# YiZhiXiaoGuLI/xerus

Measured on AMD Instinct MI355X. Metric: GFLOP/s on TT contraction + TT-round sweep time, order-10 rank-256, higher is better.
Workload: dtype f64; 1 GPU; TT order-10 n=20 rank-256: <x,y> + x.round(256) per step; order=10, mode_size=20, rank=256, parallelism=replicas x1

## Files before the change

xerus_amd/csrc/smallla.hip:

```cpp
#include "smallla.hpp"

#include "reduce_dev.hpp"

#include <cstdio>

namespace xrs {

constexpr int NB = 32;
typedef double d4 __attribute__((ext_vector_type(4)));
constexpr int PMAX = 512;
constexpr int POT_THREADS = 512;

__device__ __forceinline__ double readlane_d(double v, int l) {
    union { double d; int i[2]; } u;
    u.d = v;
    u.i[0] = __builtin_amdgcn_readlane(u.i[0], l);
    u.i[1] = __builtin_amdgcn_readlane(u.i[1], l);
    return u.d;
}

__device__ __forceinline__ void potrf32_body(double* __restrict__ G, int n, double shift_rel, double* __restrict__ Dinv,
                                             int* __restrict__ status, double* __restrict__ info,
                                             const double* src = nullptr) {
    __shared__ double P[PMAX * (NB + 1)];
    __shared__ double Ds[NB][NB + 1];
    __shared__ double red[16];
    __shared__ int fail;
    const int tid = threadIdx.x, lane = tid & 63, wave = tid >> 6;
    if (src != nullptr && src != G) {
        for (int e = tid; e < n * n; e += POT_THREADS) G[e] = src[e];
        __syncthreads();
    }
    double* dummy = Dinv + size_t(n + 31) * NB + (tid & 31);
    if (tid == 0) fail = 0;
    block_trace<POT_THREADS>(G, n, red);
    const double tr = sum_from_zero<POT_THREADS / 64>(red);
    if (tid == 0 && info) info[0] = tr;
    const double shift = shift_rel * tr;
    if (shift != 0.0)
        for (int i = tid; i < n; i += POT_THREADS) G[size_t(i) * n + i] += shift;
    __syncthreads();
    for (int j0 = 0; j0 < n; j0 += NB) {
        const int jb = min(NB, n - j0);
        for (int e = tid; e < NB * NB; e += POT_THREADS) {
            const int r = e / NB, c = e % NB;
            double v = (r == c) ? 1.0 : 0.0;
            if (r < jb && c < jb && c <= r) v = G[size_t(j0 + r) * n + j0 + c];
            Ds[r][c] = v;
        }
        __syncthreads();
        if (wave == 0) {
            const int r = lane & 31;
            double row[NB];
#pragma unroll
            for (int c = 0; c < NB; ++c) row[c] = Ds[r][c];
            int bad = 0;
#pragma unroll
            for (int k = 0; k < NB; ++k) {
                double dkk = readlane_d(row[k], k);
                const bool okp = (dkk > 0.0) && (dkk < 1.0e300);
                if (!okp && bad == 0 && k < jb) bad = k + 1;
                if (!okp) dkk = 1.0;
                const double d = sqrt(dkk);
                const double inv = 1.0 / d;
                row[k] = (r == k) ? d : ((r > k) ? row[k] * inv : row[k]);
#pragma unroll
                for (int l = k + 1; l < NB; ++l) {
                    const double v = readlane_d(row[k], l);
                    if (r >= l) row[l] -= row[k] * v;
                }
            }
            if (lane < 32) {
#pragma unroll
                for (int c = 0; c < NB; ++c) Ds[r][c] = (c <= r) ? row[c] : 0.0;
            }
            if (lane == 0 && bad && fail == 0) fail = j0 + bad;
        }
        __syncthreads();
        const int t = n - j0 - jb;
        if (wave == 1) {
            const int c = lane & 31;
            double x[NB];
#pragma unroll
            for (int i = 0; i < NB; ++i) x[i] = (i == c) ? 1.0 : 0.0;
#pragma unroll
            for (int k = 0; k < NB; ++k) {
                x[k] = x[k] / Ds[k][k];
// ... 272 lines not shown
        for (int q = 0; q < 4; ++q) {
            const int er = min(max(16 * i + lg + 4 * q, 0), n - 1), ec = min(max(16 * k + lr, 0), n - 1);
            const int row = max(er, ec), col = min(er, ec);
            acc[s][q] = S[size_t(row) * n + col];
        }
    }
#pragma unroll
    for (int s = 0; s < PR_SLOTS; ++s)
#pragma unroll
        for (int q = 0; q < 4; ++q) {
            const int row = 16 * ti[s] + lg + 4 * q, col = 16 * tk[s] + lr;
            const bool inside = ti[s] >= 0 && row < n && col < n;
            const double pad = (row == col) ? 1.0 : 0.0;
            acc[s][q] = inside ? acc[s][q] + ((row == col) ? shift : 0.0) : pad;
        }

    for (int j = 0; j < T; ++j) {
        int oc = (lg * PT + lr) * 8, oa = (lr * PT + lg) * 8;
        asm volatile("" : "+v"(oc), "+v"(oa));
        auto cpos = [&](double* base, int q) -> double* {
            return reinterpret_cast<double*>(reinterpret_cast<char*>(base) + oc) + 4 * q * PT;
        };
        auto apos = [&](const double* base, int c) -> const double* {
            return reinterpret_cast<const double*>(reinterpret_cast<const char*>(base) + oa) + 4 * c;
        };
#pragma unroll
        for (int s = 0; s < PR_SLOTS; ++s)
            if (ti[s] == j && tk[s] == j) {
#pragma unroll
                for (int q = 0; q < 4; ++q) *cpos(Dt, q) = acc[s][q];
            }
        __syncthreads();
        PSTAMP(2 + 4 * j);
        if (wave == 0) {
            const int bad = diag_factor16(Dt, Di, ivs, Dinv + size_t(j) * 256, lane, n - 16 * j);
            if (lane == 0 && bad && fail == 0) fail = 16 * j + bad;
        }
        __syncthreads();
        PSTAMP(3 + 4 * j);
#pragma unroll
        for (int s = 0; s < PR_SLOTS; ++s) {
            if (tk[s] != j) continue;
            if (ti[s] == j) {
#pragma unroll
                for (int q = 0; q < 4; ++q) acc[s][q] = *cpos(Dt, q);
                continue;
            }
            double* Pi = P + ti[s] * PTILE;
#pragma unroll
            for (int q = 0; q < 4; ++q) *cpos(Pi, q) = acc[s][q];
            wave_lds_sync();
            d4 rr = {0.0, 0.0, 0.0, 0.0};
#pragma unroll
            for (int c = 0; c < 4; ++c) rr = __builtin_amdgcn_mfma_f64_16x16x4f64(*apos(Pi, c), *apos(Di, c), rr, 0, 0, 0);
            wave_lds_sync();
#pragma unroll
            for (int q = 0; q < 4; ++q) *cpos(Pi, q) = rr[q];
            acc[s] = rr;
        }
        __syncthreads();
        PSTAMP(4 + 4 * j);
        trail_all<PR_SLOTS - 1>(acc, ti, tk, j, P, oa);
    }
    __syncthreads();
    PSTAMP(1);
    int sg = lg, sr = lr;
    asm volatile("" : "+v"(sg), "+v"(sr));
#pragma unroll
    for (int s = 0; s < PR_SLOTS; ++s) {
        if (ti[s] < 0 || G == nullptr) continue;
#pragma unroll
        for (int q = 0; q < 4; ++q) {
            const int row = 16 * ti[s] + sg + 4 * q, col = 16 * tk[s] + sr;
            if (row < n && col < n) {
                G[size_t(row) * n + col] = (col <= row) ? acc[s][q] : 0.0;
                if (ti[s] != tk[s]) G[size_t(col) * n + row] = 0.0;
            }
        }
    }
    __syncthreads();
    if (tid == 0) status[0] = fail;
}

constexpr int LA_THREADS = PR_THREADS;
constexpr int LA_WAVES = LA_THREADS / 64;
constexpr int LA_SLOTS = PR_SLOTS;

template <int P>
__device__ __forceinline__ void la_trail_pair(d4 (&acc)[LA_SLOTS], const int (&ti)[LA_SLOTS], const int (&tk)[LA_SLOTS],
                                              int kmin, int kmax, const double* Pbuf, int oa) {
    const bool hi = tk[P] >= kmin && tk[P] <= kmax;
    bool lo = false;
    if constexpr (P > 0) lo = tk[P - 1] >= kmin && tk[P - 1] <= kmax;
    if (!hi && !lo) return;
    auto op = [&](int tile, int c) -> double {
        return *reinterpret_cast<const double*>(reinterpret_cast<const char*>(Pbuf + max(tile, 0) * PTILE) + oa + 32 * c);
    };
    double a1[4], b1[4];
#pragma unroll
    for (int c = 0; c < 4; ++c) {
        a1[c] = hi ? -op(ti[P], c) : 0.0;
        b1[c] = hi ? op(tk[P], c) : 0.0;
    }
    if constexpr (P > 0) {
        double a0[4], b0[4];
#pragma unroll
        for (int c = 0; c < 4; ++c) {
            a0[c] = lo ? -op(ti[P - 1], c) : 0.0;
            b0[c] = lo ? op(tk[P - 1], c) : 0.0;
        }
#pragma unroll
        for (int c = 0; c < 4; ++c) {
            acc[P] = __builtin_amdgcn_mfma_f64_16x16x4f64(a1[c], b1[c], acc[P], 0, 0, 0);
            acc[P - 1] = __builtin_amdgcn_mfma_f64_16x16x4f64(a0[c], b0[c], acc[P - 1], 0, 0, 0);
        }
    } else {
#pragma unroll
        for (int c = 0; c < 4; ++c) acc[P] = __builtin_amdgcn_mfma_f64_16x16x4f64(a1[c], b1[c], acc[P], 0, 0, 0);
    }
}

template <int P>
__device__ __forceinline__ void la_trail_all(d4 (&acc)[LA_SLOTS], const int (&ti)[LA_SLOTS], const int (&tk)[LA_SLOTS],
                                             int kmin, int kmax, const double* Pbuf, int oa) {
    if constexpr (P >= 0) {
        la_trail_pair<P>(acc, ti, tk, kmin, kmax, Pbuf, oa);
        la_trail_all<P - 2>(acc, ti, tk, kmin, kmax, Pbuf, oa);
    }
}

__device__ __forceinline__ void potrf_la_body(double* __restrict__ G, int n, double shift_rel, double* __restrict__ Dinv,
                                              int* __restrict__ status, double* __restrict__ info,
                                              const double* __restrict__ src = nullptr) {
    const double* __restrict__ S = src != nullptr ? src : G;
    __shared__ double Dt[PTILE];
    __shared__ double Di[PTILE];
    __shared__ double P[PR_TMAX * PTILE];
    __shared__ double ivs[16];
    __shared__ double red[LA_WAVES];
    __shared__ int fail;
    const int tid = threadIdx.x, lane = tid & 63;
    const int wave = __builtin_amdgcn_readfirstlane(tid >> 6);
    const int lr = lane & 15, lg = lane >> 4;
    const int T = (n + 15) >> 4;
    const int ntiles = T * (T + 1) / 2;
    if (tid == 0) fail = 0;
    PSTAMP(0);
    block_trace<LA_THREADS>(S, n, red);
    const double tr = sum_from_zero<LA_WAVES>(red);
    if (tid == 0 && info) info[0] = tr;
    const double shift = shift_rel * tr;

    int ti[LA_SLOTS], tk[LA_SLOTS];
    d4 acc[LA_SLOTS];
#pragma unroll
    for (int s = 0; s < LA_SLOTS; ++s) {
        const int t = wave == 0 ? s : LA_SLOTS + s * (LA_WAVES - 1) + (wave - 1);
        int i = -1, k = -1;
        if (t < ntiles) {
            int start = 0;
            k = 0;
            while (t >= start + (T - k)) { start += T - k; ++k; }
            i = k + (t - start);
        }
        ti[s] = i;
        tk[s] = k;
#pragma unroll
        for (int q = 0; q < 4; ++q) {
            const int er = min(max(16 * i + lg + 4 * q, 0), n - 1), ec = min(max(16 * k + lr, 0), n - 1);
            const int row = max(er, ec), col = min(er, ec);
            acc[s][q] = S[size_t(row) * n + col];
        }
    }
#pragma unroll
    for (int s = 0; s < LA_SLOTS; ++s)
#pragma unroll
        for (int q = 0; q < 4; ++q) {
            const int row = 16 * ti[s] + lg + 4 * q, col = 16 * tk[s] + lr;
            const bool inside = ti[s] >= 0 && row < n && col < n;
            const double pad = (row == col) ? 1.0 : 0.0;
            acc[s][q] = inside ? acc[s][q] + ((row == col) ? shift : 0.0) : pad;
        }

    int oc = (lg * PT + lr) * 8, oa = (lr * PT + lg) * 8;
    auto cpos = [&](double* base, int q) -> double* {
        return reinterpret_cast<double*>(reinterpret_cast<char*>(base) + oc) + 4 * q * PT;
    };
    auto apos = [&](const double* base, int c) -> const double* {
        return reinterpret_cast<const double*>(reinterpret_cast<const char*>(base) + oa) + 4 * c;
    };
    auto publish_diag = [&](int j) {
#pragma unroll
        for (int s = 0; s < LA_SLOTS; ++s)
            if (ti[s] == j && tk[s] == j) {
#pragma unroll
                for (int q = 0; q < 4; ++q) *cpos(Dt, q) = acc[s][q];
            }
    };
    auto factor_diag = [&](int j) {
        if (wave == 0) {
            const int bad = diag_factor16(Dt, Di, ivs, Dinv + size_t(j) * 256, lane, n - 16 * j);
            if (lane == 0 && bad && fail == 0) fail = 16 * j + bad;
        }
    };
    publish_diag(0);
    __syncthreads();
    factor_diag(0);
    __syncthreads();
    for (int j = 0; j < T; ++j) {
        asm volatile("" : "+v"(oc), "+v"(oa));
        PSTAMP(2 + 4 * j);
#pragma unroll
        for (int s = 0; s < LA_SLOTS; ++s) {
            if (tk[s] != j) continue;
            if (ti[s] == j) {
#pragma unroll
                for (int q = 0; q < 4; ++q) acc[s][q] = *cpos(Dt, q);
                continue;
            }
            double* Pi = P + ti[s] * PTILE;
#pragma unroll
            for (int q = 0; q < 4; ++q) *cpos(Pi, q) = acc[s][q];
            wave_lds_sync();
            d4 rr = {0.0, 0.0, 0.0, 0.0};
#pragma unroll
            for (int c = 0; c < 4; ++c) rr = __builtin_amdgcn_mfma_f64_16x16x4f64(*apos(Pi, c), *apos(Di, c), rr, 0, 0, 0);
            wave_lds_sync();
#pragma unroll
            for (int q = 0; q < 4; ++q) *cpos(Pi, q) = rr[q];
            acc[s] = rr;
        }
        __syncthreads();
        if (j + 1 >= T) break;
        PSTAMP(3 + 4 * j);
        la_trail_all<LA_SLOTS - 1>(acc, ti, tk, j + 1, j + 1, P, oa);
        publish_diag(j + 1);
        __syncthreads();
        PSTAMP(4 + 4 * j);
        if (wave == 0) factor_diag(j + 1);
        la_trail_all<LA_SLOTS - 1>(acc, ti, tk, j + 2, T - 1, P, oa);
        __syncthreads();
    }
    PSTAMP(1);
    int sg = lg, sr = lr;
    asm volatile("" : "+v"(sg), "+v"(sr));
#pragma unroll
    for (int s = 0; s < LA_SLOTS; ++s) {
        if (ti[s] < 0 || G == nullptr) continue;
#pragma unroll
        for (int q = 0; q < 4; ++q) {
            const int row = 16 * ti[s] + sg + 4 * q, col = 16 * tk[s] + sr;
            if (row < n && col < n) {
                G[size_t(row) * n + col] = (col <= row) ? acc[s][q] : 0.0;
                if (ti[s] != tk[s]) G[size_t(col) * n + row] = 0.0;
            }
        }
    }
    __syncthreads();
    if (tid == 0) status[0] = fail;
}

#ifdef XRS_POTRF_NO_LOOKAHEAD
#define XRS_POTRF_RR_BODY potrf_rr_body
#else
#define XRS_POTRF_RR_BODY potrf_la_body
#endif
#define XRS_POTRF_RR_THREADS PR_THREADS
__global__ void __launch_bounds__(XRS_POTRF_RR_THREADS) k_potrf_rr(double* __restrict__ G, int n, double shift_rel,
                                                         double* __restrict__ Dinv, int* __restrict__ status,
                                                         double* __restrict__ info) {
    XRS_POTRF_RR_BODY(G, n, shift_rel, Dinv, status, info);
}

__global__ void __launch_bounds__(POT_THREADS) k_potrf32_batched(PotrfBatch b) {
    const int i = blockIdx.x;
    potrf32_body(b.G[i], b.n[i], b.shift[i], b.Dinv[i], b.status + b.slot[i], nullptr, b.src[i]);
}

__global__ void __launch_bounds__(XRS_POTRF_RR_THREADS) k_potrf_rr_batched(PotrfBatch b) {
    const int i = blockIdx.x;
    XRS_POTRF_RR_BODY(b.G[i], b.n[i], b.shift[i], b.Dinv[i], b.status + b.slot[i], nullptr, b.src[i]);
}

template <bool COLS, int TMAX>
__device__ __forceinline__ void trsm16_body(const double* __restrict__ L, const double* __restrict__ Dinv, int dld,
                                            int n, const double* __restrict__ Y, size_t ldy, double* __restrict__ X,
                                            size_t ldx, int nvec, int v0, bool ident) {
    constexpr int JS = TMAX / 4;
    __shared__ double Xs[TMAX * 16 * PT];
    __shared__ double red[2][4][256];
    const int tid = threadIdx.x, lane = tid & 63;
    const int wave = __builtin_amdgcn_readfirstlane(tid >> 6);
    const int lr = lane & 15, lg = lane >> 4;
    const int T = (n + 15) >> 4;
    const int np = T * 16;
    for (int e = tid; e < np * 16; e += 256) {
        int i, v;
        if (COLS) { i = e >> 4; v = e & 15; } else { v = e / np; i = e - v * np; }
        double y = 0.0;
        if (i < n && v0 + v < nvec) {
            if (ident) y = (i == v0 + v) ? 1.0 : 0.0;
            else y = COLS ? Y[size_t(i) * ldy + v0 + v] : Y[size_t(v0 + v) * ldy + i];
        }
        Xs[i * PT + v] = y;
    }
    auto dinv_at = [&](int I, int c) -> double {
        const int off = (dld == 32) ? 16 * (I & 1) : 0;
        return Dinv[size_t(16 * I + lr) * dld + off + 4 * c + lg];
    };
    d4 xr[JS];
    double la[JS][4], lb[JS][4], da[4], db[4];
#pragma unroll
    for (int js = 0; js < JS; ++js) {
        xr[js] = d4{0.0, 0.0, 0.0, 0.0};
#pragma unroll
        for (int c = 0; c < 4; ++c) la[js][c] = 0.0;
    }
#pragma unroll
    for (int c = 0; c < 4; ++c) da[c] = dinv_at(0, c);
    __syncthreads();
    for (int I = 0; I < T; ++I) {
        if (I + 1 < T) {
            const int row = 16 * (I + 1) + lr;
#pragma unroll
            for (int js = 0; js < JS; ++js) {
                const int J = wave + 4 * js;
#pragma unroll
                for (int c = 0; c < 4; ++c)
                    lb[js][c] = (J <= I && row < n) ? L[size_t(row) * n + 16 * J + 4 * c + lg] : 0.0;
            }
#pragma unroll
            for (int c = 0; c < 4; ++c) db[c] = dinv_at(I + 1, c);
        }
        d4 y;
#pragma unroll
        for (int q = 0; q < 4; ++q) y[q] = Xs[(16 * I + lg + 4 * q) * PT + lr];
        d4 accj[JS];
#pragma unroll
        for (int js = 0; js < JS; ++js) {
            accj[js] = d4{0.0, 0.0, 0.0, 0.0};
            if (wave + 4 * js >= I) continue;
#pragma unroll
            for (int c = 0; c < 4; ++c) accj[js] = __builtin_amdgcn_mfma_f64_16x16x4f64(la[js][c], xr[js][c], accj[js], 0, 0, 0);
        }
        d4 acc = accj[0];
#pragma unroll
        for (int js = 1; js < JS; ++js) acc += accj[js];
        double* rb = red[I & 1][0];
#pragma unroll
        for (int q = 0; q < 4; ++q) rb[wave * 256 + q * 64 + lane] = acc[q];
        __syncthreads();
        d4 t;
#pragma unroll
        for (int q = 0; q < 4; ++q)
            t[q] = y[q] - ((rb[q * 64 + lane] + rb[256 + q * 64 + lane]) + (rb[512 + q * 64 + lane] + rb[768 + q * 64 + lane]));
        d4 x0 = {0.0, 0.0, 0.0, 0.0}, x1 = {0.0, 0.0, 0.0, 0.0};
        x0 = __builtin_amdgcn_mfma_f64_16x16x4f64(da[0], t[0], x0, 0, 0, 0);
        x1 = __builtin_amdgcn_mfma_f64_16x16x4f64(da[1], t[1], x1, 0, 0, 0);
        x0 = __builtin_amdgcn_mfma_f64_16x16x4f64(da[2], t[2], x0, 0, 0, 0);
        x1 = __builtin_amdgcn_mfma_f64_16x16x4f64(da[3], t[3], x1, 0, 0, 0);
        const d4 x = x0 + x1;
        if ((I & 3) == wave) {
#pragma unroll
            for (int js = 0; js < JS; ++js)
// ... 225 lines not shown
        __syncthreads();
        for (int round = 0; round < P - 1; ++round) {
            for (int t = wave; t < P / 2; t += 16) {
                int i = perm[t], j = perm[P - 1 - t];
                if (i >= p || j >= p) continue;
                if (i > j) { const int s = i; i = j; j = s; }
                double* wi = W + size_t(i) * q;
                double* wj = W + size_t(j) * q;
                double a = 0, b = 0, c = 0;
                for (int k = lane; k < q; k += 64) {
                    const double x = wi[k], y = wj[k];
                    a += x * x; b += y * y; c += x * y;
                }
                a = wave_sum(a); b = wave_sum(b); c = wave_sum(c);
                if (fabs(c) > tol * sqrt(a * b) && c != 0.0) {
                    const double zeta = (b - a) / (2.0 * c);
                    const double t_ = copysign(1.0, zeta) / (fabs(zeta) + sqrt(1.0 + zeta * zeta));
                    const double cs = 1.0 / sqrt(1.0 + t_ * t_);
                    const double sn = cs * t_;
                    const double tau = sn / (1.0 + cs);
                    for (int k = lane; k < q; k += 64) {
                        const double x = wi[k], y = wj[k];
                        wi[k] = x - sn * (y + tau * x);
                        wj[k] = y + sn * (x - tau * y);
                    }
                    double* ji = J + size_t(i) * p;
                    double* jj = J + size_t(j) * p;
                    for (int k = lane; k < p; k += 64) {
                        const double x = ji[k], y = jj[k];
                        ji[k] = x - sn * (y + tau * x);
                        jj[k] = y + sn * (x - tau * y);
                    }
                    if (lane == 0) rotated = 1;
                }
            }
            __syncthreads();
            if (tid == 0) {
                const int last = perm[P - 1];
                for (int s = P - 1; s > 1; --s) perm[s] = perm[s - 1];
                perm[1] = last;
            }
            __syncthreads();
        }
        if (!rotated) break;
    }
    if (tid == 0) sweeps_out[0] = (sweep < max_sweeps) ? sweep + 1 : -1;
}

__global__ void __launch_bounds__(1024) k_svd_finish(const double* __restrict__ Wr, int p, int q, const double* __restrict__ J,
                                                      double* __restrict__ U, double* __restrict__ S, double* __restrict__ Vt) {
    __shared__ double sn[PMAX];
    __shared__ int rk[PMAX];
    const int tid = threadIdx.x, lane = tid & 63, wave = tid >> 6;
    for (int i = wave; i < p; i += 16) {
        const double* w = Wr + size_t(i) * q;
        double s = 0.0;
        for (int k = lane; k < q; k += 64) s += w[k] * w[k];
        s = wave_sum(s);
        if (lane == 0) sn[i] = sqrt(s);
    }
    __syncthreads();
    for (int i = tid; i < p; i += 1024) {
        int r = 0;
        const double si = sn[i];
        for (int j = 0; j < p; ++j) r += (sn[j] > si) || (sn[j] == si && j < i);
        rk[i] = r;
    }
    __syncthreads();
    for (int i = tid; i < p; i += 1024) S[rk[i]] = sn[i];
    for (int e = tid; e < p * q; e += 1024) {
        const int i = e / q, k = e % q;
        const double s = sn[i];
        Vt[size_t(rk[i]) * q + k] = (s > 0.0) ? Wr[e] / s : 0.0;
    }
    for (int e = tid; e < p * p; e += 1024) {
        const int i = e / p, r = e % p;
        U[size_t(r) * p + rk[i]] = J[e];
    }
}

static int dinv_ld(int n) { return n <= PR_TMAX * 16 ? 16 : 32; }
size_t dinv_elems(int n) { return dinv_ld(n) == 16 ? size_t((n + 15) / 16) * 256 : size_t(n + 32) * 32; }

void potrf(xrs_handle_t h, double* G, int n, double shift_rel, double* Dinv, int* status_dev, double* info_dev) {
    XRS_REQUIRE(n >= 1 && n <= PMAX, "potrf: n out of range for the single-workgroup kernel");
    KernelTimer timer(h, XRS_KFAM_QR, double(n) * n * n / 3.0, 16.0 * double(n) * n);
    if (dinv_ld(n) == 16) {
        hipLaunchKernelGGL(k_potrf_rr, dim3(1), dim3(XRS_POTRF_RR_THREADS), 0, h->stream, G, n, shift_rel, Dinv, status_dev, info_dev);
        check_launch("k_potrf_rr");
    } else {
        hipLaunchKernelGGL(k_potrf, dim3(1), dim3(POT_THREADS), 0, h->stream, G, n, shift_rel, Dinv, status_dev, info_dev);
        check_launch("k_potrf");
    }
}

void potrf_batched(xrs_handle_t h, const PotrfBatch& b, int count) {
    XRS_REQUIRE(count >= 0 && count <= kPotrfBatchMax, "potrf_batched: batch too large");
    if (count == 0) return;
    PotrfBatch small{}, large{};
    int ns = 0, nl = 0;
    double fl_s = 0.0, fl_l = 0.0;
    for (int i = 0; i < count; ++i) {
        XRS_REQUIRE(b.n[i] >= 1 && b.n[i] <= PMAX, "potrf_batched: n out of range");
        const bool rr = dinv_ld(b.n[i]) == 16;
        PotrfBatch& d = rr ? small : large;
        int& c = rr ? ns : nl;
        XRS_REQUIRE(b.G[i] != nullptr || (rr && b.src[i] != nullptr), "potrf_batched: no input / output");
        d.src[c] = b.src[i];
        d.G[c] = b.G[i];
        d.Dinv[c] = b.Dinv[i];
        d.shift[c] = b.shift[i];
        d.n[c] = b.n[i];
        d.slot[c] = i;
        (rr ? fl_s : fl_l) += double(b.n[i]) * b.n[i] * b.n[i] / 3.0;
        ++c;
    }
    small.status = b.status;
    large.status = b.status;
    if (ns) {
        KernelTimer timer(h, XRS_KFAM_QR, fl_s, 0.0);
        hipLaunchKernelGGL(k_potrf_rr_batched, dim3(ns), dim3(XRS_POTRF_RR_THREADS), 0, h->stream, small);
        check_launch("k_potrf_rr_batched");
    }
    if (nl) {
        KernelTimer timer(h, XRS_KFAM_QR, fl_l, 0.0);
        hipLaunchKernelGGL(k_potrf32_batched, dim3(nl), dim3(POT_THREADS), 0, h->stream, large);
        check_launch("k_potrf32_batched");
    }
}

void trsm(xrs_handle_t h, bool cols, const double* L, const double* Dinv, int n, const double* Y, size_t ldy, double* X,
          size_t ldx, int nvec) {
    if (nvec <= 0) return;
    XRS_REQUIRE(n >= 1 && n <= PMAX, "trsm: n out of range");
    KernelTimer timer(h, XRS_KFAM_QR, double(n) * n * nvec, 8.0 * (2.0 * double(n) * nvec + double(n) * n));
    const unsigned blocks = unsigned((nvec + 15) / 16);
    const int dld = dinv_ld(n);
#define XRS_TRSM(C_, T_) \
    hipLaunchKernelGGL((k_trsm16<C_, T_>), dim3(blocks), dim3(256), 0, h->stream, L, Dinv, dld, n, Y, ldy, X, ldx, nvec)
    if (n <= 256) {
        if (cols) XRS_TRSM(true, 16); else XRS_TRSM(false, 16);
    } else {
        if (cols) XRS_TRSM(true, 32); else XRS_TRSM(false, 32);
    }
#undef XRS_TRSM
    check_launch("k_trsm16");
}

void trinv_batched(xrs_handle_t h, const TrinvBatch& b, int count) {
    XRS_REQUIRE(count >= 0 && count <= kTrinvBatchMax, "trinv_batched: batch too large");
    for (int big = 0; big < 2; ++big) {
        TrinvBatch g{};
        int c = 0, nmax = 0;
        double fl = 0.0;
        for (int i = 0; i < count; ++i) {
            XRS_REQUIRE(b.n[i] >= 1 && b.n[i] <= PMAX, "trinv_batched: n out of range");
            if ((dinv_ld(b.n[i]) == 32) != bool(big)) continue;
            g.L[c] = b.L[i];
            g.Dinv[c] = b.Dinv[i];
            g.X[c] = b.X[i];
            g.n[c] = b.n[i];
            nmax = std::max(nmax, b.n[i]);
            fl += double(b.n[i]) * b.n[i] * b.n[i];
            ++c;
        }
        if (c == 0) continue;
        KernelTimer timer(h, XRS_KFAM_QR, fl, 0.0);
        const dim3 grid(unsigned((nmax + 15) / 16), unsigned(c));
        if (big) hipLaunchKernelGGL((k_trinv_batched<32>), grid, dim3(256), 0, h->stream, g, 32);
        else hipLaunchKernelGGL((k_trinv_batched<16>), grid, dim3(256), 0, h->stream, g, 16);
        check_launch("k_trinv_batched");
    }
}

size_t qrcp(xrs_handle_t h, const double* A, size_t m, size_t n, double* Q, double* C, bool pivot, bool abs_r00,
            bool rank_rule) {
    XRS_REQUIRE(m >= 1 && n >= 1, "qrcp: empty matrix");
    XRS_REQUIRE(m < (1u << 24) && n < (1u << 24), "qrcp: matrix too large");
    const size_t kmax = std::min(m, n);
    DevBuf W(h, m * n * 8), vn(h, 2 * n * 8), jp(h, n * 4 + 64), tau(h, kmax * 8), rk(h, 64);
    transpose(h, W.d(), A, m, n);
    {
        KernelTimer timer(h, XRS_KFAM_QR, 4.0 * double(m) * n * kmax, 8.0 * 4.0 * double(m) * n);
        hipLaunchKernelGGL(k_qrcp, dim3(1), dim3(1024), 0, h->stream, W.d(), int(m), int(n), vn.d(), vn.d() + n, jp.as<int>(),
                           tau.d(), Q, C, rk.as<int>(), int(pivot), int(abs_r00), int(rank_rule));
        check_launch("k_qrcp");
    }
    int r = 0;
    read_status(h, rk.as<int>(), 1, &r);
    return size_t(r);
}

void jacobi_svd_rows(xrs_handle_t h, const double* W, int p, int q, double* U, double* S, double* Vt) {
    XRS_REQUIRE(p >= 1 && p <= PMAX && p <= q, "jacobi_svd_rows: need 1 <= p <= min(q, 512)");
    DevBuf st(h, 64);
    auto one_workgroup = [&](int) {
        DevBuf Wc(h, size_t(p) * q * 8), J(h, size_t(p) * p * 8);
        XRS_HIP(hipMemcpyAsync(Wc.d(), W, size_t(p) * q * 8, hipMemcpyDeviceToDevice, h->stream));
        KernelTimer timer(h, XRS_KFAM_SVD, 8.0 * double(p) * p * (p + q), 0.0);
        hipLaunchKernelGGL(k_jacobi, dim3(1), dim3(1024), 0, h->stream, Wc.d(), p, q, J.d(), 60, 4.0 * 2.220446049250313e-16,
                           st.as<int>());
        check_launch("k_jacobi");
        hipLaunchKernelGGL(k_svd_finish, dim3(1), dim3(1024), 0, h->stream, Wc.d(), p, q, J.d(), U, S, Vt);
        check_launch("k_svd_finish");
// ... 8 lines not shown
```

xerus_amd/csrc/tt.hip:

```cpp
#include <algorithm>
#include <atomic>
#include <chrono>
#include <condition_variable>
#include <limits>
#include <memory>
#include <mutex>
#include <thread>
#include <cstdio>
#include <cstdlib>
#include <cmath>
#include <string>
#include <vector>

#include "cholqr.hpp"
#include "reduce_dev.hpp"
#include "tt_common.hpp"

namespace xrs {

namespace ttd {


std::vector<size_t> maximal_ranks(const TT& t) {
    std::vector<size_t> rk(t.r + 1, t.r + t.d);
// ... 80 lines not shown
__global__ void k_soft_cols(double* __restrict__ T, const double* __restrict__ S, size_t rows, size_t cols, double soft) {
    for (size_t e = size_t(blockIdx.x) * blockDim.x + threadIdx.x; e < rows * cols; e += size_t(gridDim.x) * blockDim.x) {
        const double s = S[e % cols];
        T[e] = s > 0.0 ? T[e] * (fmax(0.0, s - soft) / s) : 0.0;
    }
}

void truncate_edge(TT& t, size_t k, size_t max_rank, double eps, double soft) {
    const size_t m = t.r[k], nn = t.cols_right(k);
    const size_t prow = t.rows_left(k - 1);
    xrs_handle_t h = t.h;
    const bool wide = m <= nn;
    const size_t g = wide ? m : nn;
    XRS_REQUIRE(g <= kHugeMax, "TT round: an edge whose unfoldings both exceed 1024 is not supported");
    double* Q = t.alloc(m * nn);
    double* F = t.alloc(g * g);
    const OrthResult o = orthogonalize(h, t.core[k], m, nn, wide, Q, F);
    if (wide && o.certified && eps < 0.5 * o.cert_ratio && max_rank >= m && !(soft > 0.0)) {
        double* prv = t.alloc(prow * m);
        gemm(h, prv, prow, m, 1.0, t.core[k - 1], m, false, m, F, m, false);
        t.release(F);
        t.replace(k, Q);
        t.replace(k - 1, prv);
        return;
    }
    DevBuf S(h, g * 8), Vt(h, g * g * 8), st(h, 64);
    XRS_HIP(hipMemsetAsync(st.d(), 0, 64, h->stream));
    jacobi_right_vectors(h, F, int(g), wide, S.d(), Vt.d(), st.as<int>(), 60);
    jacobi_settle(h, st.as<int>(), int(g), int(g), [&](int kernel) {
        jacobi_vt(h, F, int(g), false, int(g), int(g), S.d(), Vt.d(), int(g), st.as<int>(), 60, kernel);
    });
    std::vector<double> s(g);
    XRS_HIP(hipMemcpyAsync(s.data(), S.d(), g * 8, hipMemcpyDeviceToHost, h->stream));
    host_wait(h);
    const size_t kk = svd_cut(s, max_rank, eps);
    double* T = t.alloc(m * kk);
    if (wide) gemm(h, T, m, kk, 1.0, F, g, false, g, Vt.d(), g, true);
    else gemm(h, T, m, kk, 1.0, t.core[k], nn, false, nn, Vt.d(), g, true);
    if (soft > 0.0) {
        hipLaunchKernelGGL(k_soft_cols, dim3(unsigned(std::min<size_t>((m * kk + 255) / 256, 4096))), dim3(256), 0, h->stream, T, S.d(), m, kk,
                           soft);
        check_launch("k_soft_cols");
    }
    double* cur = t.alloc(kk * nn);
    if (wide) gemm(h, cur, kk, nn, 1.0, Vt.d(), g, false, g, Q, nn, false);
    else XRS_HIP(hipMemcpyAsync(cur, Vt.d(), kk * nn * 8, hipMemcpyDeviceToDevice, h->stream));
    double* prv = t.alloc(prow * kk);
    gemm(h, prv, prow, kk, 1.0, t.core[k - 1], m, false, m, T, kk, false);
    t.release(T);
    t.release(F);
    t.release(Q);
    t.replace(k, cur);
    t.replace(k - 1, prv);
    t.r[k] = kk;
}


void left_gram_step(TT& t, std::vector<double*>& G, double* T, size_t k, bool do_reduce) {
    xrs_handle_t h = t.h;
    if (k == 0) {
        gemm_sym(h, G[1], t.r[1], 1.0, t.core[0], t.r[1], true, t.rows_left(0), t.core[0], t.r[1], false);
        if (do_reduce) t.reduce(G[1], t.r[1] * t.r[1]);
        return;
    }
    const size_t a = t.r[k], b = t.r[k + 1], cols = t.cols_right(k);
    gemm(h, T, a, cols, 1.0, G[k], a, false, a, t.core[k], cols, false);
    gemm_sym(h, G[k + 1], b, 1.0, t.core[k], b, true, a * t.n[k], T, b, false);
    if (do_reduce) t.reduce(G[k + 1], b * b);
}

void right_gram_step(TT& t, std::vector<double*>& H, double* T, size_t k, bool do_reduce) {
    xrs_handle_t h = t.h;
    const size_t last = t.d - 1;
    if (k == last) {
        const size_t cl = t.cols_right(last);
        gemm_sym(h, H[last], t.r[last], 1.0, t.core[last], cl, false, cl, t.core[last], cl, true);
        if (do_reduce) t.reduce(H[last], t.r[last] * t.r[last]);
        return;
    }
    const size_t a = t.r[k], b = t.r[k + 1], cols = t.cols_right(k);
    gemm(h, T, a * t.n[k], b, 1.0, t.core[k], b, false, b, H[k + 1], b, false);
    gemm_sym(h, H[k], a, 1.0, t.core[k], cols, false, cols, T, cols, true);
    if (do_reduce) t.reduce(H[k], a * a);
}

void gram_chains(TT& t, std::vector<double*>& G, std::vector<double*>& H, std::vector<DevBuf>& store, bool left) {
    const size_t d = t.d;
    xrs_handle_t h = t.h;
    G.assign(d, nullptr);
    H.assign(d, nullptr);
    size_t tmax = 1;
    for (size_t k = 1; k + 1 < d; ++k) tmax = std::max(tmax, t.size(k));
    DevBuf TL(h, tmax * 8), TR(h, tmax * 8);
    if (t.sharded()) {
        for (size_t s = 0; s + 1 < d; ++s) {
            const size_t kl = s + 1, kr = d - 1 - s;
            const size_t nl = left ? t.r[kl] * t.r[kl] : 0, nr = t.r[kr] * t.r[kr];
            store.emplace_back(h, (nl + nr) * 8);
            double* base = store.back().d();
            if (left) G[kl] = base;
            H[kr] = base + nl;
            if (left) {
                StreamFork fork(h);
                fork.side();
                left_gram_step(t, G, TL.d(), s, false);
                fork.main();
                right_gram_step(t, H, TR.d(), kr, false);
                fork.join();
            } else {
                right_gram_step(t, H, TR.d(), kr, false);
            }
            t.reduce(base, nl + nr);
        }
        return;
    }
    for (size_t k = 1; k < d; ++k) {
        if (left) {
            store.emplace_back(h, t.r[k] * t.r[k] * 8);
            G[k] = store.back().d();
        }
        store.emplace_back(h, t.r[k] * t.r[k] * 8);
        H[k] = store.back().d();
    }
    if (!left) {
        for (size_t k = d - 1; k >= 1; --k) right_gram_step(t, H, TR.d(), k);
        return;
    }
    StreamFork fork(h);
    for (size_t s = 0; s + 1 < d; ++s) {
        fork.side();
        left_gram_step(t, G, TL.d(), s);
        fork.main();
        right_gram_step(t, H, TR.d(), d - 1 - s);
    }
    fork.join();
}

struct HostMarks {
    bool on = stamps_enabled("round");
    std::chrono::steady_clock::time_point t0 = std::chrono::steady_clock::now();
    std::string line;
    void mark(const char* what) {
        if (!on) return;
        const double us = std::chrono::duration<double, std::micro>(std::chrono::steady_clock::now() - t0).count();
        char buf[64];
        std::snprintf(buf, sizeof(buf), " %s %.0f", what, us);
        line += buf;
    }
    HostMarks();
    ~HostMarks();
};
thread_local HostMarks* g_marks = nullptr;
HostMarks::HostMarks() { g_marks = on ? this : nullptr; }
HostMarks::~HostMarks() {
    g_marks = nullptr;
    if (on) std::fprintf(stderr, "[round host us]%s\n", line.c_str());
}
#define XRS_MARK(what) do { if (g_marks) g_marks->mark(what); } while (0)


__global__ void __launch_bounds__(256) k_dev_identity_many(const DevIdArgs args) {
    const double* G = args.G[blockIdx.x];
    const int n = args.n[blockIdx.x];
    __shared__ double red[4];
    double mx = 0.0;
    for (int e = threadIdx.x + 256 * blockIdx.y; e < n * n; e += 256 * gridDim.y) {
        const double v = fabs(G[e] - ((e / n) == (e % n) ? 1.0 : 0.0));
        mx = (v > mx || v != v) ? v : mx;
    }
    mx = block_max_nan_t0(mx, red);
    if (threadIdx.x == 0) args.out[blockIdx.x * gridDim.y + blockIdx.y] = mx;
}

void rl_sweep(TT& t, const size_t* max_ranks, double eps, double cX, size_t from);


static bool same_shape(const GemmJob& o, const GemmJob& g) {
    return o.M == g.M && o.N == g.N && o.K == g.K && o.lda == g.lda && o.ldb == g.ldb && o.ta == g.ta && o.tb == g.tb &&
           o.sym == g.sym && o.alpha == g.alpha && o.tri == g.tri;
}

std::vector<bool> largest_group(const std::vector<GemmJob>& jobs) {
    std::vector<bool> done(jobs.size(), false), best(jobs.size(), false);
    double best_flops = -1.0;
    for (size_t i = 0; i < jobs.size(); ++i) {
        if (done[i]) continue;
        std::vector<bool> mine(jobs.size(), false);
        double flops = 0.0;
        for (size_t j = i; j < jobs.size(); ++j) {
            if (done[j] || !same_shape(jobs[j], jobs[i])) continue;
            done[j] = mine[j] = true;
            flops += double(jobs[j].M) * double(jobs[j].N) * double(jobs[j].K);
        }
        if (flops > best_flops) {
            best_flops = flops;
            best = mine;
        }
    }
    return best;
}

void gemm_grouped(xrs_handle_t h, const std::vector<GemmJob>& jobs) {
    std::vector<bool> done(jobs.size(), false);
    for (size_t i = 0; i < jobs.size(); ++i) {
        if (done[i]) continue;
        const GemmJob& g = jobs[i];
        std::vector<const double*> A, B;
        std::vector<double*> C;
        for (size_t j = i; j < jobs.size(); ++j) {
            const GemmJob& o = jobs[j];
            if (done[j] || !same_shape(o, g))
                continue;
            done[j] = true;
            A.push_back(o.A);
            B.push_back(o.B);
            C.push_back(o.C);
// ... 811 lines not shown
```

Before: 37800 GFLOP/s.

## Add critical-path lookahead Cholesky with per-wave panel ownership and early dot gate

Replaces the lookahead Cholesky body with a version where a rotating wave factors the next panel tile and updates the next diagonal, double-buffering the diagonal tiles so wave 0 can factor block j+1 while the other waves apply the trailing update. Tile-to-wave assignment is reworked to put critical-path tiles on dedicated slots. The intent is to shorten the serial diagonal-factor chain inside the single-workgroup potrf. Separately, the gram chain now opens a dot gate partway through the sweep, at a step chosen by flop count, so downstream work can start earlier. The old body stays reachable through an environment variable.

```diff
diff --git a/xerus_amd/csrc/smallla.hip b/xerus_amd/csrc/smallla.hip
--- a/xerus_amd/csrc/smallla.hip
+++ b/xerus_amd/csrc/smallla.hip
@@ -3,6 +3,8 @@
 #include "reduce_dev.hpp"
 
 #include <cstdio>
+#include <cstdlib>
+#include <cstring>
 
 namespace xrs {
 
@@ -441,16 +443,17 @@
     if (tid == 0) status[0] = fail;
 }
 
-constexpr int LA_THREADS = PR_THREADS;
-constexpr int LA_WAVES = LA_THREADS / 64;
-constexpr int LA_SLOTS = PR_SLOTS;
+constexpr int CF_THREADS = PR_THREADS;
+constexpr int CF_WAVES = CF_THREADS / 64;
+constexpr int CF_SLOTS = PR_SLOTS;
+constexpr int CF_CRIT = 6;
 
 template <int P>
-__device__ __forceinline__ void la_trail_pair(d4 (&acc)[LA_SLOTS], const int (&ti)[LA_SLOTS], const int (&tk)[LA_SLOTS],
-                                              int kmin, int kmax, const double* Pbuf, int oa) {
-    const bool hi = tk[P] >= kmin && tk[P] <= kmax;
+__device__ __forceinline__ void cf_trail_pair(d4 (&acc)[CF_SLOTS], const int (&ti)[CF_SLOTS], const int (&tk)[CF_SLOTS],
+                                              int kmin, int imin, const double* Pbuf, int oa) {
+    const bool hi = tk[P] >= kmin && ti[P] >= imin;
     bool lo = false;
-    if constexpr (P > 0) lo = tk[P - 1] >= kmin && tk[P - 1] <= kmax;
+    if constexpr (P > 0) lo = tk[P - 1] >= kmin && ti[P - 1] >= imin;
     if (!hi && !lo) return;
     auto op = [&](int tile, int c) -> double {
         return *reinterpret_cast<const double*>(reinterpret_cast<const char*>(Pbuf + max(tile, 0) * PTILE) + oa + 32 * c);
@@ -480,47 +483,73 @@
 }
 
 template <int P>
-__device__ __forceinline__ void la_trail_all(d4 (&acc)[LA_SLOTS], const int (&ti)[LA_SLOTS], const int (&tk)[LA_SLOTS],
-                                             int kmin, int kmax, const double* Pbuf, int oa) {
+__device__ __forceinline__ void cf_trail_all(d4 (&acc)[CF_SLOTS], const int (&ti)[CF_SLOTS], const int (&tk)[CF_SLOTS],
+                                             int kmin, int imin, const double* Pbuf, int oa) {
     if constexpr (P >= 0) {
-        la_trail_pair<P>(acc, ti, tk, kmin, kmax, Pbuf, oa);
-        la_trail_all<P - 2>(acc, ti, tk, kmin, kmax, Pbuf, oa);
-    }
-}
-
-__device__ __forceinline__ void potrf_la_body(double* __restrict__ G, int n, double shift_rel, double* __restrict__ Dinv,
+        cf_trail_pair<P>(acc, ti, tk, kmin, imin, Pbuf, oa);
+        cf_trail_all<P - 2>(acc, ti, tk, kmin, imin, Pbuf, oa);
+    }
+}
+
+__device__ __forceinline__ void potrf_cf_body(double* __restrict__ G, int n, double shift_rel, double* __restrict__ Dinv,
                                               int* __restrict__ status, double* __restrict__ info,
                                               const double* __restrict__ src = nullptr) {
     const double* __restrict__ S = src != nullptr ? src : G;
-    __shared__ double Dt[PTILE];
-    __shared__ double Di[PTILE];
+    __shared__ double Dt2[2 * PTILE];
+    __shared__ double Di2[2 * PTILE];
     __shared__ double P[PR_TMAX * PTILE];
     __shared__ double ivs[16];
-    __shared__ double red[LA_WAVES];
+    __shared__ double red[CF_WAVES];
     __shared__ int fail;
     const int tid = threadIdx.x, lane = tid & 63;
     const int wave = __builtin_amdgcn_readfirstlane(tid >> 6);
     const int lr = lane & 15, lg = lane >> 4;
     const int T = (n + 15) >> 4;
-    const int ntiles = T * (T + 1) / 2;
     if (tid == 0) fail = 0;
     PSTAMP(0);
-    block_trace<LA_THREADS>(S, n, red);
-    const double tr = sum_from_zero<LA_WAVES>(red);
+    block_trace<CF_THREADS>(S, n, red);
+    const double tr = sum_from_zero<CF_WAVES>(red);
     if (tid == 0 && info) info[0] = tr;
     const double shift = shift_rel * tr;
 
-    int ti[LA_SLOTS], tk[LA_SLOTS];
-    d4 acc[LA_SLOTS];
-#pragma unroll
-    for (int s = 0; s < LA_SLOTS; ++s) {
-        const int t = wave == 0 ? s : LA_SLOTS + s * (LA_WAVES - 1) + (wave - 1);
+    int ti[CF_SLOTS], tk[CF_SLOTS];
+    d4 acc[CF_SLOTS];
+    const int ncrit = wave == 1 ? CF_CRIT : CF_CRIT - 2;
+#pragma unroll
+    for (int s = 0; s < CF_SLOTS; ++s) {
         int i = -1, k = -1;
-        if (t < ntiles) {
-            int start = 0;
-            k = 0;
-            while (t >= start + (T - k)) { start += T - k; ++k; }
-            i = k + (t - start);
+        if (wave == 0) {
+            if (s == 0) {
+                i = 0;
+                k = 0;
+            } else if (s < PR_TMAX - 1) {
+                if (s + 1 < T) {
+                    i = s + 1;
+                    k = 0;
+                }
+            } else if (s - 12 < T) {
+                i = s - 12;
+                k = 1;
+            }
+        } else if (s < ncrit) {
+            const int jc = wave - 1 + (CF_WAVES - 1) * (s >> 1);
+            if (jc + 1 < T) {
+                i = jc + 1;
+                k = (s & 1) ? jc + 1 : jc;
+            }
+        } else {
+            const int sp = s - ncrit;
+            int rho = sp < 11 ? sp * (CF_WAVES - 1) + wave - 1 : 11 * (CF_WAVES - 1) + (sp - 11) * (CF_WAVES - 2) + wave - 2;
+            int kk = 1, i0 = 5;
+            while (kk < T && rho >= max(T - i0, 0)) {
+                rho -= max(T - i0, 0);
+                ++kk;
+                i0 = kk + 2;
+            }
+            if (kk < T) {
+                k = kk;
+                i = i0 + rho;
+            }
         }
         ti[s] = i;
         tk[s] = k;
@@ -528,14 +557,16 @@
         for (int q = 0; q < 4; ++q) {
             const int er = min(max(16 * i + lg + 4 * q, 0), n - 1), ec = min(max(16 * k + lr, 0), n - 1);
             const int row = max(er, ec), col = min(er, ec);
-            acc[s][q] = S[size_t(row) * n + col];
-        }
-    }
-#pragma unroll
-    for (int s = 0; s < LA_SLOTS; ++s)
+            acc[s][q] = *reinterpret_cast<const double*>(reinterpret_cast<const char*>(S) + unsigned(row * n + col) * 8u);
+        }
+    }
+    int fg = lg, fr = lr;
+    asm volatile("" : "+v"(fg), "+v"(fr));
+#pragma unroll
+    for (int s = 0; s < CF_SLOTS; ++s)
 #pragma unroll
         for (int q = 0; q < 4; ++q) {
-            const int row = 16 * ti[s] + lg + 4 * q, col = 16 * tk[s] + lr;
+            const int row = 16 * ti[s] + fg + 4 * q, col = 16 * tk[s] + fr;
             const bool inside = ti[s] >= 0 && row < n && col < n;
             const double pad = (row == col) ? 1.0 : 0.0;
             acc[s][q] = inside ? acc[s][q] + ((row == col) ? shift : 0.0) : pad;
@@ -548,63 +579,82 @@
     auto apos = [&](const double* base, int c) -> const double* {
         return reinterpret_cast<const double*>(reinterpret_cast<const char*>(base) + oa) + 4 * c;
     };
-    auto publish_diag = [&](int j) {
-#pragma unroll
-        for (int s = 0; s < LA_SLOTS; ++s)
-            if (ti[s] == j && tk[s] == j) {
-#pragma unroll
-                for (int q = 0; q < 4; ++q) *cpos(Dt, q) = acc[s][q];
-            }
+    auto panel_tile = [&](d4& a, int i, const double* Di) {
+        double* Pi = P + i * PTILE;
+#pragma unroll
+        for (int q = 0; q < 4; ++q) *cpos(Pi, q) = a[q];
+        wave_lds_sync();
+        d4 rr = {0.0, 0.0, 0.0, 0.0};
+#pragma unroll
+        for (int c = 0; c < 4; ++c) rr = __builtin_amdgcn_mfma_f64_16x16x4f64(*apos(Pi, c), *apos(Di, c), rr, 0, 0, 0);
+        wave_lds_sync();
+#pragma unroll
+        for (int q = 0; q < 4; ++q) *cpos(Pi, q) = rr[q];
+        a = rr;
     };
     auto factor_diag = [&](int j) {
-        if (wave == 0) {
-            const int bad = diag_factor16(Dt, Di, ivs, Dinv + size_t(j) * 256, lane, n - 16 * j);
-            if (lane == 0 && bad && fail == 0) fail = 16 * j + bad;
-        }
+        double* Dt = Dt2 + (j & 1) * PTILE;
+        double* Di = Di2 + (j & 1) * PTILE;
+        const int bad = diag_factor16(Dt, Di, ivs, Dinv + size_t(j) * 256, lane, n - 16 * j);
+        if (lane == 0 && bad && fail == 0) fail = 16 * j + bad;
     };
-    publish_diag(0);
-    __syncthreads();
-    factor_diag(0);
-    __syncthreads();
+    if (wave == 0) {
+#pragma unroll
+        for (int q = 0; q < 4; ++q) *cpos(Dt2, q) = acc[0][q];
+    }
+    __syncthreads();
+    if (wave == 0) factor_diag(0);
     for (int j = 0; j < T; ++j) {
         asm volatile("" : "+v"(oc), "+v"(oa));
+        double* Dt = Dt2 + (j & 1) * PTILE;
+        double* Di = Di2 + (j & 1) * PTILE;
+        double* Dn = Dt2 + ((j + 1) & 1) * PTILE;
+        __syncthreads();
         PSTAMP(2 + 4 * j);
-#pragma unroll
-        for (int s = 0; s < LA_SLOTS; ++s) {
-            if (tk[s] != j) continue;
+        if (j + 1 < T) {
+            if (wave == 1 + j % (CF_WAVES - 1)) {
+#pragma unroll
+                for (int s = 0; s < CF_CRIT; s += 2) {
+                    if (ti[s] != j + 1 || tk[s] != j || tk[s + 1] != j + 1) continue;
+                    panel_tile(acc[s], j + 1, Di);
+                    wave_lds_sync();
+                    const double* Pi = P + (j + 1) * PTILE;
+                    double b[4];
+#pragma unroll
+                    for (int c = 0; c < 4; ++c) b[c] = *apos(Pi, c);
+#pragma unroll
+                    for (int c = 0; c < 4; ++c)
+                        acc[s + 1] = __builtin_amdgcn_mfma_f64_16x16x4f64(-b[c], b[c], acc[s + 1], 0, 0, 0);
+#pragma unroll
+                    for (int q = 0; q < 4; ++q) *cpos(Dn, q) = acc[s + 1][q];
+                }
+            }
+        }
+#pragma unroll
+        for (int s = 0; s < CF_SLOTS; ++s) {
+            if (tk[s] != j || ti[s] == j + 1) continue;
             if (ti[s] == j) {
 #pragma unroll
                 for (int q = 0; q < 4; ++q) acc[s][q] = *cpos(Dt, q);
                 continue;
             }
-            double* Pi = P + ti[s] * PTILE;
-#pragma unroll
-            for (int q = 0; q < 4; ++q) *cpos(Pi, q) = acc[s][q];
-            wave_lds_sync();
-            d4 rr = {0.0, 0.0, 0.0, 0.0};
-#pragma unroll
-            for (int c = 0; c < 4; ++c) rr = __builtin_amdgcn_mfma_f64_16x16x4f64(*apos(Pi, c), *apos(Di, c), rr, 0, 0, 0);
-            wave_lds_sync();
-#pragma unroll
-            for (int q = 0; q < 4; ++q) *cpos(Pi, q) = rr[q];
-            acc[s] = rr;
-        }
-        __syncthreads();
+            panel_tile(acc[s], ti[s], Di);
+        }
         if (j + 1 >= T) break;
+        __syncthreads();
         PSTAMP(3 + 4 * j);
-        la_trail_all<LA_SLOTS - 1>(acc, ti, tk, j + 1, j + 1, P, oa);
-        publish_diag(j + 1);
-        __syncthreads();
-        PSTAMP(4 + 4 * j);
-        if (wave == 0) factor_diag(j + 1);
-        la_trail_all<LA_SLOTS - 1>(acc, ti, tk, j + 2, T - 1, P, oa);
-        __syncthreads();
-    }
+        if (wave == 0) {
+            factor_diag(j + 1);
+            PSTAMP(4 + 4 * j);
+        }
+        if (wave != 0 || j == 0) cf_trail_all<CF_SLOTS - 1>(acc, ti, tk, j + 1, j + 2, P, oa);
+    }
+    __syncthreads();
     PSTAMP(1);
     int sg = lg, sr = lr;
     asm volatile("" : "+v"(sg), "+v"(sr));
 #pragma unroll
-    for (int s = 0; s < LA_SLOTS; ++s) {
+    for (int s = 0; s < CF_SLOTS; ++s) {
         if (ti[s] < 0 || G == nullptr) continue;
 #pragma unroll
         for (int q = 0; q < 4; ++q) {
@@ -619,16 +669,17 @@
     if (tid == 0) status[0] = fail;
 }
 
-#ifdef XRS_POTRF_NO_LOOKAHEAD
-#define XRS_POTRF_RR_BODY potrf_rr_body
-#else
-#define XRS_POTRF_RR_BODY potrf_la_body
-#endif
 #define XRS_POTRF_RR_THREADS PR_THREADS
 __global__ void __launch_bounds__(XRS_POTRF_RR_THREADS) k_potrf_rr(double* __restrict__ G, int n, double shift_rel,
                                                          double* __restrict__ Dinv, int* __restrict__ status,
                                                          double* __restrict__ info) {
-    XRS_POTRF_RR_BODY(G, n, shift_rel, Dinv, status, info);
+    potrf_cf_body(G, n, shift_rel, Dinv, status, info);
+}
+
+__global__ void __launch_bounds__(XRS_POTRF_RR_THREADS) k_potrf_rr_plain(double* __restrict__ G, int n, double shift_rel,
+                                                               double* __restrict__ Dinv, int* __restrict__ status,
+                                                               double* __restrict__ info) {
+    potrf_rr_body(G, n, shift_rel, Dinv, status, info);
 }
 
 __global__ void __launch_bounds__(POT_THREADS) k_potrf32_batched(PotrfBatch b) {
@@ -638,7 +689,12 @@
 
 __global__ void __launch_bounds__(XRS_POTRF_RR_THREADS) k_potrf_rr_batched(PotrfBatch b) {
     const int i = blockIdx.x;
-    XRS_POTRF_RR_BODY(b.G[i], b.n[i], b.shift[i], b.Dinv[i], b.status + b.slot[i], nullptr, b.src[i]);
+    potrf_cf_body(b.G[i], b.n[i], b.shift[i], b.Dinv[i], b.status + b.slot[i], nullptr, b.src[i]);
+}
+
+__global__ void __launch_bounds__(XRS_POTRF_RR_THREADS) k_potrf_rr_plain_batched(PotrfBatch b) {
+    const int i = blockIdx.x;
+    potrf_rr_body(b.G[i], b.n[i], b.shift[i], b.Dinv[i], b.status + b.slot[i], nullptr, b.src[i]);
 }
 
 template <bool COLS, int TMAX>
@@ -1030,11 +1086,19 @@
 static int dinv_ld(int n) { return n <= PR_TMAX * 16 ? 16 : 32; }
 size_t dinv_elems(int n) { return dinv_ld(n) == 16 ? size_t((n + 15) / 16) * 256 : size_t(n + 32) * 32; }
 
+static bool potrf_plain_body() {
+    const char* e = std::getenv("XRS_POTRF_BODY");
+    return e && std::strcmp(e, "plain") == 0;
+}
+
 void potrf(xrs_handle_t h, double* G, int n, double shift_rel, double* Dinv, int* status_dev, double* info_dev) {
     XRS_REQUIRE(n >= 1 && n <= PMAX, "potrf: n out of range for the single-workgroup kernel");
     KernelTimer timer(h, XRS_KFAM_QR, double(n) * n * n / 3.0, 16.0 * double(n) * n);
     if (dinv_ld(n) == 16) {
-        hipLaunchKernelGGL(k_potrf_rr, dim3(1), dim3(XRS_POTRF_RR_THREADS), 0, h->stream, G, n, shift_rel, Dinv, status_dev, info_dev);
+        if (potrf_plain_body())
+            hipLaunchKernelGGL(k_potrf_rr_plain, dim3(1), dim3(XRS_POTRF_RR_THREADS), 0, h->stream, G, n, shift_rel, Dinv, status_dev, info_dev);
+        else
+            hipLaunchKernelGGL(k_potrf_rr, dim3(1), dim3(XRS_POTRF_RR_THREADS), 0, h->stream, G, n, shift_rel, Dinv, status_dev, info_dev);
         check_launch("k_potrf_rr");
     } else {
         hipLaunchKernelGGL(k_potrf, dim3(1), dim3(POT_THREADS), 0, h->stream, G, n, shift_rel, Dinv, status_dev, info_dev);
@@ -1067,7 +1131,10 @@
     large.status = b.status;
     if (ns) {
         KernelTimer timer(h, XRS_KFAM_QR, fl_s, 0.0);
-        hipLaunchKernelGGL(k_potrf_rr_batched, dim3(ns), dim3(XRS_POTRF_RR_THREADS), 0, h->stream, small);
+        if (potrf_plain_body())
+            hipLaunchKernelGGL(k_potrf_rr_plain_batched, dim3(ns), dim3(XRS_POTRF_RR_THREADS), 0, h->stream, small);
+        else
+            hipLaunchKernelGGL(k_potrf_rr_batched, dim3(ns), dim3(XRS_POTRF_RR_THREADS), 0, h->stream, small);
         check_launch("k_potrf_rr_batched");
     }
     if (nl) {
diff --git a/xerus_amd/csrc/tt.hip b/xerus_amd/csrc/tt.hip
--- a/xerus_amd/csrc/tt.hip
+++ b/xerus_amd/csrc/tt.hip
@@ -186,6 +186,24 @@
     gemm(h, T, a * t.n[k], b, 1.0, t.core[k], b, false, b, H[k + 1], b, false);
     gemm_sym(h, H[k], a, 1.0, t.core[k], cols, false, cols, T, cols, true);
     if (do_reduce) t.reduce(H[k], a * a);
+}
+
+static size_t dot_gate_step(const TT& t) {
+    const size_t d = t.d;
+    int early = 2;
+    if (const char* e = std::getenv("XRS_DOT_GATE_EARLY"); e && e[0] >= '0' && e[0] <= '9' && e[1] == 0) early = e[0] - '0';
+    if (early == 0 || d < 3) return d;
+    auto flops = [&](size_t k) { return double(t.r[k]) * double(t.n[k]) * double(t.r[k + 1]) * double(t.r[k] + t.r[k + 1]); };
+    auto step = [&](size_t s) { return std::max(flops(s), flops(d - 1 - s)); };
+    double top = 0.0;
+    for (size_t s = 0; s + 1 < d; ++s) top = std::max(top, step(s));
+    size_t at = d;
+    for (size_t s = d - 1; s-- > 0;) {
+        if (step(s) * 4.0 < top) continue;
+        at = s;
+        if (--early == 0) break;
+    }
+    return at + 2 == d ? d : at;
 }
 
 void gram_chains(TT& t, std::vector<double*>& G, std::vector<double*>& H, std::vector<DevBuf>& store, bool left) {
@@ -230,12 +248,14 @@
         for (size_t k = d - 1; k >= 1; --k) right_gram_step(t, H, TR.d(), k);
         return;
     }
+    const size_t gate_step = dot_gate_step(t);
     StreamFork fork(h);
     for (size_t s = 0; s + 1 < d; ++s) {
         fork.side();
         left_gram_step(t, G, TL.d(), s);
         fork.main();
         right_gram_step(t, H, TR.d(), d - 1 - s);
+        if (s == gate_step) open_dot_gate(h);
     }
     fork.join();
 }
```

Result: faster. 40220 GFLOP/s (median of 6 runs) (+6.4%).
